# lucasjinreal/yolov7_d2

Hardware: NVIDIA H100
Metric: images/sec (640x640) YOLOX-s fwd+bwd (higher is better)
Workload: dtype bf16

## Files before the change

yolov7_d2_b200/csrc/conv_api.cu:

```cuda
#include "conv_gemm.cuh"
#include "host_common.cuh"
#include "wgrad_gemm.cuh"

#include <algorithm>
#include <cstring>

namespace yb {

template <int BN, int BK>
static int launch_conv_inst(const CUtensorMap& tmA, const CUtensorMap& tmB, const ConvGemmParams& p, dim3 grid, cudaStream_t st) {
  using Cfg = ConvGemmCfg<BN, BK>;
  const bool ext = p.epi_mode >= EPI_BF16_AFFINE;
  const int phases = p.num_phases == 4 ? 4 : 1;
  const int m_tiles = grid.x * phases, n_tiles = grid.y;
  const int occ = conv_min_ctas(BN, BK);
  const bool xpose = p.epi_mode == EPI_F32_BIAS && p.out_sc == 1;
  const int fixed = ConvEpiCfg<BN>::kStageBytes + (xpose ? kXposeBytes : 0);
  const int budget = (occ == 1 ? 212 : 104) * 1024 - 1024 - fixed;
  int slots_kb = budget / Cfg::kStageBytes;
  const int num_kb = phases == 4 ? p.cin_blocks : p.num_taps * p.cin_blocks;
  int kbs = 1;
  if (BK <= 32)
    for (int t = 1; t <= num_kb; ++t)
      if (num_kb % t == 0 && t * BK <= 144 && 2 * t <= slots_kb) kbs = t;
  int pst = slots_kb / kbs;
  if (pst > kMaxStagesP) pst = kMaxStagesP;
  if (pst < 2) pst = 2;
  const int smem = pst * kbs * Cfg::kStageBytes + 1024 + fixed;
  static PerDevice<int> smem_limit(0);
  YB_CHECK_CUDA(raise_smem_limit(smem_limit, smem, conv_gemm_persistent_kernel<BN, BK, false>, conv_gemm_persistent_kernel<BN, BK, true>));
  int groups = (occ * sm_count()) / n_tiles;
  if (groups < 1) groups = 1;
  if (groups > m_tiles) groups = m_tiles;
  if (phases == 4 && groups > 1 && groups % 2 == 0) --groups;
  ConvGemmParams pp = p;
  pp.xpose = xpose ? 1 : 0;
  if (ext)
    launch_k(conv_gemm_persistent_kernel<BN, BK, true>, groups * n_tiles, kConvThreadsP, smem, st, tmA, tmB, pp, pst, kbs, n_tiles, m_tiles);
  else
    launch_k(conv_gemm_persistent_kernel<BN, BK, false>, groups * n_tiles, kConvThreadsP, smem, st, tmA, tmB, pp, pst, kbs, n_tiles, m_tiles);
  YB_CHECK_CUDA(cudaGetLastError());
  return 0;
}

static int launch_conv(int bn, int bk, const CUtensorMap& tmA, const CUtensorMap& tmB, const ConvGemmParams& p, dim3 grid, cudaStream_t st) {
#define YB_CASE(BN, BK) \
  if (bn == BN && bk == BK) return launch_conv_inst<BN, BK>(tmA, tmB, p, grid, st);
  YB_CASE(16, 16) YB_CASE(16, 32) YB_CASE(16, 64)
  YB_CASE(32, 16) YB_CASE(32, 32) YB_CASE(32, 64)
  YB_CASE(64, 16) YB_CASE(64, 32) YB_CASE(64, 64)
  YB_CASE(128, 16) YB_CASE(128, 32) YB_CASE(128, 64)
#undef YB_CASE
  return fail(YB200_ERR_UNSUPPORTED, "no conv_gemm instantiation for BLOCK_N=%d BLOCK_K=%d", bn, bk);
}

static int pick_block_k(int c) { return c % 64 == 0 ? 64 : (c % 32 == 0 ? 32 : (c % 16 == 0 ? 16 : 0)); }
static int pick_block_n(int c) { return c > 64 ? 128 : (c > 32 ? 64 : (c > 16 ? 32 : 16)); }

static int check_arg(const yb200_act* a, const char* who, const char* arg) {
  char name[96];
  snprintf(name, sizeof(name), "%s %s", who, arg);
  return check_act(a, name);
}
// ... 676 lines not shown
```

yolov7_d2_b200/csrc/conv_gemm.cuh:

```cuda
#pragma once
#include <cuda_fp16.h>

#include "sm90.cuh"

namespace yb {

constexpr int kMaxTaps = 54;

enum EpiMode : int {
  EPI_BF16 = 0,
  EPI_F16 = 1,
  EPI_F16_STATS = 2,
  EPI_F32_BIAS = 3,
  EPI_BF16_BN_SILU = 4,
  EPI_BF16_AFFINE = 5,
  EPI_BF16_BIAS_GELU = 6,
  EPI_BF16_GELU_BWD = 7,
  EPI_BF16_BIAS_RELU = 8,
  EPI_BF16_RELU_BWD = 9,
};

__device__ __forceinline__ bool epi_has_stats(int mode, const double* stat_sum) {
  return mode == EPI_F16_STATS || ((mode == EPI_BF16_GELU_BWD || mode == EPI_BF16_RELU_BWD) && stat_sum != nullptr);
}
// ... 59 lines not shown
    ntaps = p.phase_tap[ph + 1] - tap0;
    oph = ph >> 1;
    opw = ph & 1;
  } else {
    m = wi; tap0 = 0; ntaps = p.num_taps; oph = opw = 0;
  }
}

template <int BLOCK_N, int BLOCK_K>
struct ConvGemmCfg {
  static constexpr int kSwizzle = BLOCK_K * 2;
  static constexpr int kABytes = 128 * BLOCK_K * 2;
  static constexpr int kBBytes = BLOCK_N * BLOCK_K * 2;
  static constexpr int kStageBytes = kABytes + kBBytes;
  static_assert(BLOCK_K == 16 || BLOCK_K == 32 || BLOCK_K == 64, "BLOCK_K");
  static_assert(BLOCK_N == 16 || BLOCK_N == 32 || BLOCK_N == 64 || BLOCK_N == 128, "BLOCK_N");
  static_assert(kABytes % (8 * kSwizzle) == 0 && kStageBytes % (8 * kSwizzle) == 0, "tiles must start on a swizzle-pattern boundary");
};

__device__ __forceinline__ uint32_t pack_f16x2(float lo, float hi) {
  __half2 v = __floats2half2_rn(lo, hi);
  return *reinterpret_cast<uint32_t*>(&v);
}
__device__ __forceinline__ void store_f16x8(__half* dst, const float* v) {
  uint4 u;
  u.x = pack_f16x2(v[0], v[1]);
  u.y = pack_f16x2(v[2], v[3]);
  u.z = pack_f16x2(v[4], v[5]);
  u.w = pack_f16x2(v[6], v[7]);
  *reinterpret_cast<uint4*>(dst) = u;
}
__device__ __forceinline__ void store_bf16x8(__nv_bfloat16* dst, const float* v) {
  uint4 u;
  u.x = pack_bf16x2(v[0], v[1]);
  u.y = pack_bf16x2(v[2], v[3]);
  u.z = pack_bf16x2(v[4], v[5]);
  u.w = pack_bf16x2(v[6], v[7]);
  *reinterpret_cast<uint4*>(dst) = u;
}

template <int BLOCK_N>
__device__ __forceinline__ void stage_col_params(const ConvGemmParams& p, int col0, float (*s_col)[BLOCK_N]) {
  const float* sh = p.shift ? p.shift : p.bias;
  for (int i = threadIdx.x; i < BLOCK_N; i += blockDim.x) {
    const bool ok = col0 + i < p.cout;
    s_col[0][i] = (ok && p.scale) ? p.scale[col0 + i] : 1.f;
    s_col[1][i] = (ok && sh) ? sh[col0 + i] : 0.f;
  }
}

constexpr int kXposeWarpFloats = 32 * 33 + 64;
constexpr int kXposeBytes = 8 * kXposeWarpFloats * 4;

template <int CH, bool EXT = true>
__device__ __forceinline__ void conv_epilogue_chunk(const ConvGemmParams& p, float (&v)[CH], bool valid, long long pix_off, long long add_off,
                                                    int cbase, int lane, float* part_sum, float* part_sq, bool accumulate,
                                                    const float* col_scale, const float* col_shift, float* xp = nullptr) {
  if (p.epi_mode == EPI_F32_BIAS) {
    if (xp != nullptr) {
      long long* s_off = reinterpret_cast<long long*>(xp + 32 * 33);
#pragma unroll
      for (int i = 0; i < CH; ++i) xp[lane * 33 + i] = v[i] + col_shift[i];
      s_off[lane] = valid ? pix_off : -1;
      __syncwarp();
      float* o = reinterpret_cast<float*>(p.out) + cbase + lane;
      const bool colok = lane < CH && cbase + lane < p.cout;
#pragma unroll 8
      for (int r = 0; r < 32; ++r) {
        const long long off = s_off[r];
        if (off >= 0 && colok) o[off] = xp[r * 33 + lane];
      }
      __syncwarp();
      return;
    }
    if (valid) {
      float* o = reinterpret_cast<float*>(p.out) + pix_off;
#pragma unroll
      for (int i = 0; i < CH; ++i)
        if (cbase + i < p.cout) o[(long long)(cbase + i) * p.out_sc] = v[i] + col_shift[i];
    }
    return;
  }
  if (p.epi_mode == EPI_BF16_BN_SILU) {
#pragma unroll
    for (int i = 0; i < CH; i += 4) {
      const float4 sc = *reinterpret_cast<const float4*>(col_scale + i), sh = *reinterpret_cast<const float4*>(col_shift + i);
      const float u0 = fmaf(v[i], sc.x, sh.x), u1 = fmaf(v[i + 1], sc.y, sh.y), u2 = fmaf(v[i + 2], sc.z, sh.z), u3 = fmaf(v[i + 3], sc.w, sh.w);
      v[i] = bf16_round(__fdividef(u0, 1.f + __expf(-u0)));
      v[i + 1] = bf16_round(__fdividef(u1, 1.f + __expf(-u1)));
      v[i + 2] = bf16_round(__fdividef(u2, 1.f + __expf(-u2)));
      v[i + 3] = bf16_round(__fdividef(u3, 1.f + __expf(-u3)));
    }
  }
  if constexpr (EXT) {
    if (p.epi_mode == EPI_BF16_AFFINE) {
      if (p.scale != nullptr) {
  #pragma unroll
        for (int i = 0; i < CH; i += 4) {
          const float4 sc = *reinterpret_cast<const float4*>(col_scale + i);
          v[i] *= sc.x; v[i + 1] *= sc.y; v[i + 2] *= sc.z; v[i + 3] *= sc.w;
        }
      }
      if (p.shift != nullptr) {
  #pragma unroll
        for (int i = 0; i < CH; i += 4) {
          const float4 sh = *reinterpret_cast<const float4*>(col_shift + i);
          v[i] += sh.x; v[i + 1] += sh.y; v[i + 2] += sh.z; v[i + 3] += sh.w;
        }
      }
    }
    if (p.epi_mode == EPI_BF16_BIAS_RELU) {
  #pragma unroll
      for (int i = 0; i < CH; i += 4) {
        const float4 sh = *reinterpret_cast<const float4*>(col_shift + i);
        v[i] = fmaxf(v[i] + sh.x, 0.f); v[i + 1] = fmaxf(v[i + 1] + sh.y, 0.f);
        v[i + 2] = fmaxf(v[i + 2] + sh.z, 0.f); v[i + 3] = fmaxf(v[i + 3] + sh.w, 0.f);
// ... 21 lines not shown
      }
      if (p.aux_out != nullptr && valid) {
        __nv_bfloat16* o = p.aux_out + pix_off + cbase;
  #pragma unroll
        for (int i = 0; i < CH; i += 8)
          if (cbase + i < p.cout) store_bf16x8(o + i, v + i);
      }
  #pragma unroll
      for (int i = 0; i < CH; ++i) v[i] = gelu_erf(v[i]);
    }
    if (p.epi_mode == EPI_BF16_GELU_BWD && valid) {
      const __nv_bfloat16* a = p.aux_in + pix_off + cbase;
  #pragma unroll
      for (int i = 0; i < CH; i += 8) {
        if (cbase + i < p.cout) {
          const uint4 u = *reinterpret_cast<const uint4*>(a + i);
          v[i + 0] *= gelu_erf_grad(bf16_lo(u.x)); v[i + 1] *= gelu_erf_grad(bf16_hi(u.x));
          v[i + 2] *= gelu_erf_grad(bf16_lo(u.y)); v[i + 3] *= gelu_erf_grad(bf16_hi(u.y));
          v[i + 4] *= gelu_erf_grad(bf16_lo(u.z)); v[i + 5] *= gelu_erf_grad(bf16_hi(u.z));
          v[i + 6] *= gelu_erf_grad(bf16_lo(u.w)); v[i + 7] *= gelu_erf_grad(bf16_hi(u.w));
        }
      }
    }
  }
  if (p.addend != nullptr && valid) {
    const __nv_bfloat16* a = p.addend + add_off + cbase;
#pragma unroll
    for (int i = 0; i < CH; i += 8) {
      if (cbase + i < p.cout) {
        const uint4 u = *reinterpret_cast<const uint4*>(a + i);
        v[i + 0] += bf16_lo(u.x); v[i + 1] += bf16_hi(u.x);
        v[i + 2] += bf16_lo(u.y); v[i + 3] += bf16_hi(u.y);
        v[i + 4] += bf16_lo(u.z); v[i + 5] += bf16_hi(u.z);
        v[i + 6] += bf16_lo(u.w); v[i + 7] += bf16_hi(u.w);
      }
    }
  }
  const bool f16 = p.epi_mode == EPI_F16 || p.epi_mode == EPI_F16_STATS;
  const bool need_vals = p.epi_mode == EPI_F16_STATS || (EXT && p.stat_sum != nullptr);
  if (f16) {
    uint32_t pk[CH / 2];
#pragma unroll
    for (int i = 0; i < CH; i += 2) pk[i >> 1] = pack_f16x2(v[i], v[i + 1]);
    if (valid) {
      __half* o = reinterpret_cast<__half*>(p.out) + pix_off + cbase;
#pragma unroll
      for (int i = 0; i < CH; i += 8)
        if (cbase + i < p.cout) *reinterpret_cast<uint4*>(o + i) = make_uint4(pk[i >> 1], pk[(i >> 1) + 1], pk[(i >> 1) + 2], pk[(i >> 1) + 3]);
    }
    if (need_vals) {
#pragma unroll
      for (int i = 0; i < CH; i += 2) {
        __half2 h;
        *reinterpret_cast<uint32_t*>(&h) = pk[i >> 1];
        const float2 f = __half22float2(h);
        v[i] = valid ? f.x : 0.f;
        v[i + 1] = valid ? f.y : 0.f;
      }
    }
  } else {
    uint32_t pk[CH / 2];
#pragma unroll
    for (int i = 0; i < CH; i += 2) pk[i >> 1] = pack_bf16x2(v[i], v[i + 1]);
    if (valid) {
      __nv_bfloat16* o = reinterpret_cast<__nv_bfloat16*>(p.out) + pix_off + cbase;
#pragma unroll
      for (int i = 0; i < CH; i += 8)
        if (cbase + i < p.cout) *reinterpret_cast<uint4*>(o + i) = make_uint4(pk[i >> 1], pk[(i >> 1) + 1], pk[(i >> 1) + 2], pk[(i >> 1) + 3]);
    }
    if (need_vals) {
#pragma unroll
      for (int i = 0; i < CH; i += 2) {
        v[i] = valid ? bf16_lo(pk[i >> 1]) : 0.f;
        v[i + 1] = valid ? bf16_hi(pk[i >> 1]) : 0.f;
      }
    }
  }
  if (p.epi_mode == EPI_F16_STATS) {
    float sq[CH];
#pragma unroll
    for (int i = 0; i < CH; ++i) sq[i] = v[i] * v[i];
    float cs, cq;
    if constexpr (CH == 32) { cs = warp_colsum32(v, lane); cq = warp_colsum32(sq, lane); }
    else { cs = warp_colsum16(v, lane); cq = warp_colsum16(sq, lane); }
    if (lane < CH) {
      part_sum[lane] = accumulate ? part_sum[lane] + cs : cs;
      part_sq[lane] = accumulate ? part_sq[lane] + cq : cq;
    }
  } else if (EXT && (p.epi_mode == EPI_BF16_GELU_BWD || p.epi_mode == EPI_BF16_RELU_BWD) && p.stat_sum != nullptr) {
    float cs;
    if constexpr (CH == 32) cs = warp_colsum32(v, lane);
    else cs = warp_colsum16(v, lane);
    if (lane < CH) part_sum[lane] = accumulate ? part_sum[lane] + cs : cs;
  }
}

constexpr int kMaxStagesP = 8;
constexpr int kConvThreadsP = 288;

template <int BLOCK_N>
struct ConvEpiCfg {
  static constexpr int kCols = BLOCK_N <= 64 ? (BLOCK_N < 32 ? BLOCK_N : 32) : 64;
  static_assert(BLOCK_N % kCols == 0, "staging rounds must cover the column tile");
  static constexpr int kPitch = kCols + 4;
  static constexpr int kHalves = BLOCK_N >= 32 ? 2 : 1;
  static constexpr int kChunk = kCols / kHalves;
  static constexpr int kStageBytes = 2 * 64 * kPitch * 4;
};

__host__ __device__ constexpr int conv_min_ctas(int block_n, int block_k) { return (block_n >= 128 || block_k == 16) ? 1 : 2; }

template <int BLOCK_N, int BLOCK_K, bool EXT>
__global__ void __launch_bounds__(kConvThreadsP, conv_min_ctas(BLOCK_N, BLOCK_K))
conv_gemm_persistent_kernel(const __grid_constant__ CUtensorMap tmA, const __grid_constant__ CUtensorMap tmB,
                            const __grid_constant__ ConvGemmParams p, int num_stages, int kb_per_slot, int n_tiles, int m_tiles) {
  using Cfg = ConvGemmCfg<BLOCK_N, BLOCK_K>;
  using Epi = ConvEpiCfg<BLOCK_N>;
  constexpr int CH = Epi::kChunk;
  extern __shared__ uint8_t smem_dyn[];
  __shared__ __align__(8) uint64_t s_bar[2 * kMaxStagesP];
  __shared__ float s_part[4][2][BLOCK_N];
  __shared__ __align__(16) float s_col[2][BLOCK_N];

  const int warp = warp_id_uniform();
  const int lane = threadIdx.x & 31;
  const uint32_t smem_base = (smem_u32(smem_dyn) + 1023u) & ~1023u;
  uint8_t* const smem_al = smem_dyn + (smem_base - smem_u32(smem_dyn));
  const int ring_bytes = num_stages * kb_per_slot * Cfg::kStageBytes;
  const uint32_t bar_full = smem_u32(&s_bar[0]);
  const uint32_t bar_empty = smem_u32(&s_bar[kMaxStagesP]);

  const int n_tile = blockIdx.x % n_tiles;
  const int group = blockIdx.x / n_tiles;
  const int groups = gridDim.x / n_tiles;
  const int col0 = n_tile * BLOCK_N;
  const int log_tw = p.log_tw, log_th = p.log_th;

  if (threadIdx.x == 0) {
    for (int s = 0; s < num_stages; ++s) {
      mbar_init(bar_full + 8 * s, 1);
      mbar_init(bar_empty + 8 * s, 2);
    }
    mbar_fence_init();
  }
  for (int i = threadIdx.x; i < 4 * 2 * BLOCK_N; i += blockDim.x) (&s_part[0][0][0])[i] = 0.f;
  pdl_sync();
  stage_col_params<BLOCK_N>(p, col0, s_col);
  __syncthreads();

  if (warp == 8) {
    if (elect_one()) {
      tma_prefetch_desc(&tmA);
      tma_prefetch_desc(&tmB);
      int stage = 0;
      uint32_t phase = 0;
      for (int wi = group; wi < m_tiles; wi += groups) {
        int m, tap, ntaps, oph, opw;
        conv_decode_work(p, wi, m, tap, ntaps, oph, opw);
        const int num_kb = ntaps * p.cin_blocks;
        int t = m;
        const int tw = t % p.tiles_w;
        t /= p.tiles_w;
        const int th = t % p.tiles_h;
        const int tn = t / p.tiles_h;
        const int w0 = tw << log_tw, h0 = th << log_th, n0 = tn << (7 - log_tw - log_th);
// ... 5 lines not shown
          for (int j = 0; j < kb_per_slot; ++j) {
            const uint32_t sa = smem_base + (stage * kb_per_slot + j) * Cfg::kStageBytes;
            const ConvTap& tp = p.taps[tap];
            tma_load_5d(sa, &tmA, full, tp.c0 + cb * BLOCK_K, w0 + tp.dw, tp.p, h0 + tp.dh, n0);
            tma_load_2d(sa + Cfg::kABytes, &tmB, full, tp.kb + cb * BLOCK_K, col0 + n0 * p.b_img_rows);
            if (++cb == p.cin_blocks) { cb = 0; ++tap; }
          }
          if (++stage == num_stages) { stage = 0; phase ^= 1u; }
        }
      }
    }
  } else if (warp < 8) {
    const int g = warp >> 2;
    const int wl = warp & 3;
    const int q = 2 * g + (wl & 1);
    const int half = wl >> 1;
    const int mrow = q * 32 + lane;
    const int xl = mrow & ((1 << log_tw) - 1);
    const int yl = (mrow >> log_tw) & ((1 << log_th) - 1);
    const int nl = mrow >> (log_tw + log_th);
    float* const stg = reinterpret_cast<float*>(smem_al + ring_bytes) + g * 64 * Epi::kPitch;
    float* xp = nullptr;
    if (p.xpose) xp = reinterpret_cast<float*>(smem_al + ring_bytes + Epi::kStageBytes) + warp * kXposeWarpFloats;
    constexpr uint32_t lcode = gmma_layout_code(Cfg::kSwizzle);
    constexpr uint32_t sbo = 8 * Cfg::kSwizzle;
    float acc[BLOCK_N / 2];
#pragma unroll
    for (int i = 0; i < BLOCK_N / 2; ++i) acc[i] = 0.f;
    wgmma_fence_operand(acc);
    int stage = 0;
    uint32_t phase = 0;
    for (int wi = group; wi < m_tiles; wi += groups) {
      int m, tap, ntaps, oph, opw;
      conv_decode_work(p, wi, m, tap, ntaps, oph, opw);
      const int num_kb = ntaps * p.cin_blocks;
      int j = 0, prev = -1;
      for (int kb = 0; kb < num_kb; ++kb) {
        if (j == 0) mbar_wait(bar_full + 8 * stage, phase);
        const uint32_t sa = smem_base + (stage * kb_per_slot + j) * Cfg::kStageBytes + g * 64 * Cfg::kSwizzle;
        const uint32_t sb = smem_base + (stage * kb_per_slot + j) * Cfg::kStageBytes + Cfg::kABytes;
        wgmma_fence_operand(acc);
        wgmma_fence();
#pragma unroll
        for (int k = 0; k < BLOCK_K / 16; ++k)
          Wgmma<BLOCK_N>::template mma<0, 0>(acc, gmma_desc(sa + k * 32, 16, sbo, lcode), gmma_desc(sb + k * 32, 16, sbo, lcode), (kb | k) != 0 ? 1u : 0u);
        wgmma_commit();
        wgmma_wait<1>();
        wgmma_fence_operand(acc);
        mbar_arrive_if(bar_empty + 8 * prev, j == 0 && prev >= 0 && (threadIdx.x & 127) == 0);
        if (++j == kb_per_slot) {
          j = 0;
          prev = stage;
          if (++stage == num_stages) { stage = 0; phase ^= 1u; }
        }
      }
      wgmma_wait<0>();
      wgmma_fence_operand(acc);
      mbar_arrive_if(bar_empty + 8 * prev, (threadIdx.x & 127) == 0);

      int t = m;
      const int tw = t % p.tiles_w;
      t /= p.tiles_w;
      const int th = t % p.tiles_h;
      const int tn = t / p.tiles_h;
      const int x = (tw << log_tw) + xl, y = (th << log_th) + yl, n = (tn << (7 - log_tw - log_th)) + nl;
      const bool valid = (x < p.w_valid) && (y < p.h_valid) && (n < p.n_valid);
      const long long pix_off = (long long)n * p.out_sn + (long long)(y * p.out_mh + oph) * p.out_sh +
                                (long long)(x * p.out_mw + opw) * p.out_sw;
      const long long add_off = (long long)n * p.add_sn + (long long)(y * p.out_mh + oph) * p.add_sh +
                                (long long)(x * p.out_mw + opw) * p.add_sw;
      float* const r0 = stg + (16 * wl + (lane >> 2)) * Epi::kPitch + 2 * (lane & 3);
      float* const r1 = r0 + 8 * Epi::kPitch;
      const float* const row_src = stg + ((wl & 1) * 32 + lane) * Epi::kPitch + half * CH;
#pragma unroll 1
      for (int r = 0; r < BLOCK_N / Epi::kCols; ++r) {
        named_bar_sync(1 + g, 128);
#pragma unroll
        for (int i = 0; i < BLOCK_N / 8; ++i) {
          if (i / (Epi::kCols / 8) == r) {
            const int c = (i % (Epi::kCols / 8)) * 8;
            *reinterpret_cast<float2*>(r0 + c) = make_float2(acc[4 * i], acc[4 * i + 1]);
            *reinterpret_cast<float2*>(r1 + c) = make_float2(acc[4 * i + 2], acc[4 * i + 3]);
          }
        }
        named_bar_sync(1 + g, 128);
        const int c = r * Epi::kCols + half * CH;
        if (half < Epi::kHalves && col0 + c < p.cout) {
          float v[CH];
#pragma unroll
          for (int i = 0; i < CH; i += 4) {
            const float4 f = *reinterpret_cast<const float4*>(row_src + i);
            v[i] = f.x; v[i + 1] = f.y; v[i + 2] = f.z; v[i + 3] = f.w;
          }
          conv_epilogue_chunk<CH, EXT>(p, v, valid, pix_off, add_off, col0 + c, lane, &s_part[q][0][c], &s_part[q][1][c], true, &s_col[0][c],
                                       &s_col[1][c], xp);
        }
      }
    }
  }

  __syncthreads();
  if (EXT ? epi_has_stats(p.epi_mode, p.stat_sum) : p.epi_mode == EPI_F16_STATS) {
    for (int e = threadIdx.x; e < BLOCK_N && col0 + e < p.cout; e += blockDim.x) {
      const float s1 = (s_part[0][0][e] + s_part[1][0][e]) + (s_part[2][0][e] + s_part[3][0][e]);
      const float s2 = (s_part[0][1][e] + s_part[1][1][e]) + (s_part[2][1][e] + s_part[3][1][e]);
      const int ch = p.stat_fold > 0 ? (col0 + e) % p.stat_fold : col0 + e;
      atomicAdd(p.stat_sum + ch, static_cast<double>(s1));
      if (p.stat_sq != nullptr) atomicAdd(p.stat_sq + ch, static_cast<double>(s2));
    }
  }
}

}
```

yolov7_d2_b200/csrc/host_common.cu:

```cuda
#include "host_common.cuh"

#include <mutex>

namespace yb {

static thread_local char g_err[1024] = "";

char* err_buf() { return g_err; }

int fail(int code, const char* fmt, ...) {
  va_list ap;
  va_start(ap, fmt);
  vsnprintf(g_err, sizeof(g_err), fmt, ap);
  va_end(ap);
  return code;
}

int current_device() {
  int dev = 0;
  if (cudaGetDevice(&dev) != cudaSuccess) return 0;
  return dev;
}

int sm_count() {
// ... 61 lines not shown
  YB_REQUIRE(r == CUDA_SUCCESS, YB200_ERR_CUDA,
             "cuTensorMapEncodeTiled(act n=%d h=%d w=%d pitch=%d box=%d,%d,%d,%d) failed: %d", a.n, a.h, a.w, a.c_pitch,
             box_c, tw, th, tn, static_cast<int>(r));
  return 0;
}

int make_mat_map(CUtensorMap* m, const void* ptr, long long rows, long long cols, int box_rows, int box_cols) {
  EncodeTiledFn fn = encode_fn();
  YB_REQUIRE(fn != nullptr, YB200_ERR_CUDA, "cuTensorMapEncodeTiled entry point not available");
  YB_REQUIRE((reinterpret_cast<uintptr_t>(ptr) & 15) == 0 && cols % 8 == 0, YB200_ERR_INVALID,
             "matrix must be 16B aligned with a row length multiple of 8");
  cuuint64_t gdim[2] = {static_cast<cuuint64_t>(cols), static_cast<cuuint64_t>(rows)};
  cuuint64_t gstr[1] = {static_cast<cuuint64_t>(cols) * 2};
  cuuint32_t box[2] = {static_cast<cuuint32_t>(box_cols), static_cast<cuuint32_t>(box_rows)};
  cuuint32_t estr[2] = {1, 1};
  CUresult r = fn(m, CU_TENSOR_MAP_DATA_TYPE_BFLOAT16, 2, const_cast<void*>(ptr), gdim, gstr, box, estr,
                  CU_TENSOR_MAP_INTERLEAVE_NONE, swizzle_for(box_cols * 2), CU_TENSOR_MAP_L2_PROMOTION_L2_128B,
                  CU_TENSOR_MAP_FLOAT_OOB_FILL_NONE);
  YB_REQUIRE(r == CUDA_SUCCESS, YB200_ERR_CUDA, "cuTensorMapEncodeTiled(mat %lldx%lld box %dx%d) failed: %d", rows, cols,
             box_rows, box_cols, static_cast<int>(r));
  return 0;
}

void choose_tile(int n, int h, int w, int npix, int* log_tw, int* log_th) {
  const int lp = ilog2(npix);
  long long best = -1;
  int bw = 0, bh = 0;
  for (int lw = lp; lw >= 0; --lw) {
    for (int lh = lp - lw; lh >= 0; --lh) {
      const int tw = 1 << lw, th = 1 << lh, tn = npix >> (lw + lh);
      const long long cost = 1LL * ceil_div(w, tw) * tw * ceil_div(h, th) * th * ceil_div(n, tn) * tn;
      if (best < 0 || cost < best) {
        best = cost; bw = lw; bh = lh;
      }
    }
  }
  *log_tw = bw;
  *log_th = bh;
}

}

extern "C" int yb200_version(void) { return YB200_VERSION; }
extern "C" const char* yb200_last_error(void) { return yb::err_buf(); }
```

yolov7_d2_b200/csrc/host_common.cuh:

```cuda
#pragma once
#include <cuda.h>
#include <cuda_runtime.h>
#include <stdarg.h>
#include <stdio.h>
#include <string.h>

#include <utility>

#include "../../include/yb200.h"

namespace yb {

char* err_buf();
int fail(int code, const char* fmt, ...);
int sm_count();
int current_device();
template <typename T>
struct PerDevice {
  T v[64];
  T init;
  bool used[64];
  explicit PerDevice(T init_value) : init(init_value) { memset(used, 0, sizeof(used)); }
  T& cur() {
    const int d = current_device() & 63;
// ... 10 lines not shown
  ((e = e == cudaSuccess ? cudaFuncSetAttribute(kernels, cudaFuncAttributeMaxDynamicSharedMemorySize, bytes) : e), ...);
  if (e == cudaSuccess) cur = bytes;
  return e;
}

#define YB_CHECK_CUDA(expr)                                                                      \
  do {                                                                                           \
    cudaError_t _e = (expr);                                                                     \
    if (_e != cudaSuccess) return yb::fail(YB200_ERR_CUDA, "%s: %s", #expr, cudaGetErrorString(_e)); \
  } while (0)
#define YB_REQUIRE(cond, code, ...) \
  do {                              \
    if (!(cond)) return yb::fail(code, __VA_ARGS__); \
  } while (0)

inline cudaStream_t as_stream(void* s) { return reinterpret_cast<cudaStream_t>(s); }

int check_act(const yb200_act* a, const char* name, int mult = 8);
inline bool same_shape(const yb200_act* a, const yb200_act* b) { return a->n == b->n && a->h == b->h && a->w == b->w && a->c == b->c; }
inline bool same_geometry(const yb200_act* a, const yb200_act* b) { return same_shape(a, b) && a->c_pitch == b->c_pitch; }

int make_act_map(CUtensorMap* m, const yb200_act& a, bool space_to_depth, int box_c, int tw, int th, int tn);
int make_mat_map(CUtensorMap* m, const void* ptr, long long rows, long long cols, int box_rows, int box_cols);

void choose_tile(int n, int h, int w, int npix, int* log_tw, int* log_th);

template <typename... K, typename... A>
inline cudaError_t launch_k_opt(bool pdl, void (*kernel)(K...), dim3 grid, dim3 block, size_t smem, cudaStream_t st, A&&... args) {
  cudaLaunchConfig_t cfg = {};
  cfg.gridDim = grid;
  cfg.blockDim = block;
  cfg.dynamicSmemBytes = smem;
  cfg.stream = st;
  cudaLaunchAttribute at[1];
  at[0].id = cudaLaunchAttributeProgrammaticStreamSerialization;
  at[0].val.programmaticStreamSerializationAllowed = 1;
  cfg.attrs = at;
  cfg.numAttrs = pdl ? 1 : 0;
  return cudaLaunchKernelEx(&cfg, kernel, std::forward<A>(args)...);
}
template <typename... K, typename... A>
inline cudaError_t launch_k(void (*kernel)(K...), dim3 grid, dim3 block, size_t smem, cudaStream_t st, A&&... args) {
  return launch_k_opt(true, kernel, grid, block, smem, st, std::forward<A>(args)...);
}

inline int ceil_div(int a, int b) { return (a + b - 1) / b; }
// ... 4 lines not shown
```

yolov7_d2_b200/csrc/sm90.cuh:

```cuda
#pragma once
#include <cuda.h>
#include <cuda_runtime.h>
#include <cuda_bf16.h>
#include <stdint.h>
#include <stdio.h>

namespace yb {

__device__ __forceinline__ void pdl_sync() {
  asm volatile("griddepcontrol.wait;" ::: "memory");
  asm volatile("griddepcontrol.launch_dependents;" ::: "memory");
}

__device__ __forceinline__ uint32_t smem_u32(const void* p) {
  return static_cast<uint32_t>(__cvta_generic_to_shared(p));
}

__device__ __forceinline__ bool elect_one() {
  uint32_t pred = 0;
  asm volatile(
      "{\n\t.reg .pred P;\n\t"
      "elect.sync _|P, 0xffffffff;\n\t"
      "selp.u32 %0, 1, 0, P;\n\t}\n"
      : "=r"(pred));
// ... 37 lines not shown
__device__ __forceinline__ int warp_id_uniform() { return __shfl_sync(0xffffffffu, static_cast<int>(threadIdx.x >> 5), 0); }

__device__ __forceinline__ void tma_prefetch_desc(const CUtensorMap* m) {
  asm volatile("prefetch.tensormap [%0];" ::"l"(reinterpret_cast<uint64_t>(m)) : "memory");
}
__device__ __forceinline__ void tma_load_2d(uint32_t dst, const CUtensorMap* m, uint32_t bar, int c0,
                                            int c1) {
  asm volatile(
      "cp.async.bulk.tensor.2d.shared::cluster.global.mbarrier::complete_tx::bytes [%0], [%1, {%3, "
      "%4}], [%2];"
      ::"r"(dst), "l"(reinterpret_cast<uint64_t>(m)), "r"(bar), "r"(c0), "r"(c1)
      : "memory");
}
__device__ __forceinline__ void tma_load_5d(uint32_t dst, const CUtensorMap* m, uint32_t bar, int c0,
                                            int c1, int c2, int c3, int c4) {
  asm volatile(
      "cp.async.bulk.tensor.5d.shared::cluster.global.mbarrier::complete_tx::bytes [%0], [%1, {%3, "
      "%4, %5, %6, %7}], [%2];"
      ::"r"(dst), "l"(reinterpret_cast<uint64_t>(m)), "r"(bar), "r"(c0), "r"(c1), "r"(c2), "r"(c3),
      "r"(c4)
      : "memory");
}

__device__ __forceinline__ void fence_proxy_async_smem() { asm volatile("fence.proxy.async.shared::cta;" ::: "memory"); }

__host__ __device__ constexpr uint32_t gmma_layout_code(int swizzle_bytes) {
  return swizzle_bytes == 128 ? 1u : swizzle_bytes == 64 ? 2u : swizzle_bytes == 32 ? 3u : 0u;
}
__device__ __forceinline__ uint64_t gmma_desc(uint32_t saddr, uint32_t lbo_bytes, uint32_t sbo_bytes, uint32_t layout_code) {
  uint64_t d = 0;
  d |= static_cast<uint64_t>((saddr & 0x3FFFFu) >> 4);
  d |= static_cast<uint64_t>((lbo_bytes >> 4) & 0x3FFFu) << 16;
  d |= static_cast<uint64_t>((sbo_bytes >> 4) & 0x3FFFu) << 32;
  d |= static_cast<uint64_t>(layout_code) << 62;
  return d;
}
__device__ __forceinline__ void wgmma_fence() { asm volatile("wgmma.fence.sync.aligned;" ::: "memory"); }
__device__ __forceinline__ void wgmma_commit() { asm volatile("wgmma.commit_group.sync.aligned;" ::: "memory"); }
template <int N>
__device__ __forceinline__ void wgmma_wait() { asm volatile("wgmma.wait_group.sync.aligned %0;" ::"n"(N) : "memory"); }
template <int R>
__device__ __forceinline__ void wgmma_fence_operand(float (&d)[R]) {
#pragma unroll
  for (int i = 0; i < R; ++i) asm volatile("" : "+f"(d[i])::"memory");
}

template <int N>
// ... 113 lines not shown
```

Baseline: 2037.

## Route 16-bit conv epilogue through swizzled smem with TMA stores and residual loads

Result: faster. 2332, median of 6 (+14.5%).

```diff
diff --git a/yolov7_d2_b200/csrc/conv_api.cu b/yolov7_d2_b200/csrc/conv_api.cu
--- a/yolov7_d2_b200/csrc/conv_api.cu
+++ b/yolov7_d2_b200/csrc/conv_api.cu
@@ -6,11 +6,39 @@
 #include <cstring>
 
 namespace yb {
+
+static int make_out_maps(ConvOutMaps* om, const ConvGemmParams& p, int bn) {
+  YB_REQUIRE(p.out_sc == 1, YB200_ERR_INVALID, "conv: a 16-bit output needs channel stride 1");
+  int hx, hy, hn;
+  conv_half_offset(p.log_tw, p.log_th, hx, hy, hn);
+  const int tw = 1 << p.log_tw, th = 1 << p.log_th, tn = 128 >> (p.log_tw + p.log_th);
+  const int bw = hx ? tw / 2 : tw, bh = hy ? th / 2 : th, bnn = hn ? tn / 2 : tn;
+  const int box_c = bn < 64 ? bn : 64;
+  for (int ph = 0; ph < (p.num_phases == 4 ? 4 : 1); ++ph) {
+    const int oph = ph >> 1, opw = ph & 1;
+    const char* out = static_cast<const char*>(p.out) + 2 * (oph * p.out_sh + opw * p.out_sw);
+    int rc = make_pix_map(&om->out[ph], out, p.cout, p.w_valid, p.h_valid, p.n_valid, p.out_mw * p.out_sw, p.out_mh * p.out_sh, p.out_sn, box_c,
+                          bw, bh, bnn);
+    if (rc) return rc;
+    if (p.addend == nullptr) continue;
+    const char* add = reinterpret_cast<const char*>(p.addend) + 2 * (oph * p.add_sh + opw * p.add_sw);
+    rc = make_pix_map(&om->add[ph], add, p.cout, p.w_valid, p.h_valid, p.n_valid, p.out_mw * p.add_sw, p.out_mh * p.add_sh, p.add_sn, box_c, bw,
+                      bh, bnn);
+    if (rc) return rc;
+  }
+  return 0;
+}
 
 template <int BN, int BK>
 static int launch_conv_inst(const CUtensorMap& tmA, const CUtensorMap& tmB, const ConvGemmParams& p, dim3 grid, cudaStream_t st) {
   using Cfg = ConvGemmCfg<BN, BK>;
   const bool ext = p.epi_mode >= EPI_BF16_AFFINE;
+  ConvOutMaps om;
+  memset(&om, 0, sizeof(om));
+  if (!ext && p.epi_mode != EPI_F32_BIAS) {
+    const int rc = make_out_maps(&om, p, BN);
+    if (rc) return rc;
+  }
   const int phases = p.num_phases == 4 ? 4 : 1;
   const int m_tiles = grid.x * phases, n_tiles = grid.y;
   const int occ = conv_min_ctas(BN, BK);
@@ -36,9 +64,9 @@
   ConvGemmParams pp = p;
   pp.xpose = xpose ? 1 : 0;
   if (ext)
-    launch_k(conv_gemm_persistent_kernel<BN, BK, true>, groups * n_tiles, kConvThreadsP, smem, st, tmA, tmB, pp, pst, kbs, n_tiles, m_tiles);
+    launch_k(conv_gemm_persistent_kernel<BN, BK, true>, groups * n_tiles, kConvThreadsP, smem, st, tmA, tmB, pp, om, pst, kbs, n_tiles, m_tiles);
   else
-    launch_k(conv_gemm_persistent_kernel<BN, BK, false>, groups * n_tiles, kConvThreadsP, smem, st, tmA, tmB, pp, pst, kbs, n_tiles, m_tiles);
+    launch_k(conv_gemm_persistent_kernel<BN, BK, false>, groups * n_tiles, kConvThreadsP, smem, st, tmA, tmB, pp, om, pst, kbs, n_tiles, m_tiles);
   YB_CHECK_CUDA(cudaGetLastError());
   return 0;
 }
diff --git a/yolov7_d2_b200/csrc/conv_gemm.cuh b/yolov7_d2_b200/csrc/conv_gemm.cuh
--- a/yolov7_d2_b200/csrc/conv_gemm.cuh
+++ b/yolov7_d2_b200/csrc/conv_gemm.cuh
@@ -105,14 +105,6 @@
   __half2 v = __floats2half2_rn(lo, hi);
   return *reinterpret_cast<uint32_t*>(&v);
 }
-__device__ __forceinline__ void store_f16x8(__half* dst, const float* v) {
-  uint4 u;
-  u.x = pack_f16x2(v[0], v[1]);
-  u.y = pack_f16x2(v[2], v[3]);
-  u.z = pack_f16x2(v[4], v[5]);
-  u.w = pack_f16x2(v[6], v[7]);
-  *reinterpret_cast<uint4*>(dst) = u;
-}
 __device__ __forceinline__ void store_bf16x8(__nv_bfloat16* dst, const float* v) {
   uint4 u;
   u.x = pack_bf16x2(v[0], v[1]);
@@ -137,8 +129,8 @@
 
 template <int CH, bool EXT = true>
 __device__ __forceinline__ void conv_epilogue_chunk(const ConvGemmParams& p, float (&v)[CH], bool valid, long long pix_off, long long add_off,
-                                                    int cbase, int lane, float* part_sum, float* part_sq, bool accumulate,
-                                                    const float* col_scale, const float* col_shift, float* xp = nullptr) {
+                                                    int cbase, int lane, float* part_sum, bool accumulate, const float* col_scale,
+                                                    const float* col_shift, float* xp = nullptr) {
   if (p.epi_mode == EPI_F32_BIAS) {
     if (xp != nullptr) {
       long long* s_off = reinterpret_cast<long long*>(xp + 32 * 33);
@@ -164,17 +156,6 @@
     }
     return;
   }
-  if (p.epi_mode == EPI_BF16_BN_SILU) {
-#pragma unroll
-    for (int i = 0; i < CH; i += 4) {
-      const float4 sc = *reinterpret_cast<const float4*>(col_scale + i), sh = *reinterpret_cast<const float4*>(col_shift + i);
-      const float u0 = fmaf(v[i], sc.x, sh.x), u1 = fmaf(v[i + 1], sc.y, sh.y), u2 = fmaf(v[i + 2], sc.z, sh.z), u3 = fmaf(v[i + 3], sc.w, sh.w);
-      v[i] = bf16_round(__fdividef(u0, 1.f + __expf(-u0)));
-      v[i + 1] = bf16_round(__fdividef(u1, 1.f + __expf(-u1)));
-      v[i + 2] = bf16_round(__fdividef(u2, 1.f + __expf(-u2)));
-      v[i + 3] = bf16_round(__fdividef(u3, 1.f + __expf(-u3)));
-    }
-  }
   if constexpr (EXT) {
     if (p.epi_mode == EPI_BF16_AFFINE) {
       if (p.scale != nullptr) {
@@ -242,43 +223,19 @@
         }
       }
     }
-  }
-  if (p.addend != nullptr && valid) {
-    const __nv_bfloat16* a = p.addend + add_off + cbase;
-#pragma unroll
-    for (int i = 0; i < CH; i += 8) {
-      if (cbase + i < p.cout) {
-        const uint4 u = *reinterpret_cast<const uint4*>(a + i);
-        v[i + 0] += bf16_lo(u.x); v[i + 1] += bf16_hi(u.x);
-        v[i + 2] += bf16_lo(u.y); v[i + 3] += bf16_hi(u.y);
-        v[i + 4] += bf16_lo(u.z); v[i + 5] += bf16_hi(u.z);
-        v[i + 6] += bf16_lo(u.w); v[i + 7] += bf16_hi(u.w);
-      }
-    }
-  }
-  const bool f16 = p.epi_mode == EPI_F16 || p.epi_mode == EPI_F16_STATS;
-  const bool need_vals = p.epi_mode == EPI_F16_STATS || (EXT && p.stat_sum != nullptr);
-  if (f16) {
-    uint32_t pk[CH / 2];
-#pragma unroll
-    for (int i = 0; i < CH; i += 2) pk[i >> 1] = pack_f16x2(v[i], v[i + 1]);
-    if (valid) {
-      __half* o = reinterpret_cast<__half*>(p.out) + pix_off + cbase;
-#pragma unroll
-      for (int i = 0; i < CH; i += 8)
-        if (cbase + i < p.cout) *reinterpret_cast<uint4*>(o + i) = make_uint4(pk[i >> 1], pk[(i >> 1) + 1], pk[(i >> 1) + 2], pk[(i >> 1) + 3]);
-    }
-    if (need_vals) {
-#pragma unroll
-      for (int i = 0; i < CH; i += 2) {
-        __half2 h;
-        *reinterpret_cast<uint32_t*>(&h) = pk[i >> 1];
-        const float2 f = __half22float2(h);
-        v[i] = valid ? f.x : 0.f;
-        v[i + 1] = valid ? f.y : 0.f;
-      }
-    }
-  } else {
+      if (p.addend != nullptr && valid) {
+      const __nv_bfloat16* a = p.addend + add_off + cbase;
+#pragma unroll
+      for (int i = 0; i < CH; i += 8) {
+        if (cbase + i < p.cout) {
+          const uint4 u = *reinterpret_cast<const uint4*>(a + i);
+          v[i + 0] += bf16_lo(u.x); v[i + 1] += bf16_hi(u.x);
+          v[i + 2] += bf16_lo(u.y); v[i + 3] += bf16_hi(u.y);
+          v[i + 4] += bf16_lo(u.z); v[i + 5] += bf16_hi(u.z);
+          v[i + 6] += bf16_lo(u.w); v[i + 7] += bf16_hi(u.w);
+        }
+      }
+    }
     uint32_t pk[CH / 2];
 #pragma unroll
     for (int i = 0; i < CH; i += 2) pk[i >> 1] = pack_bf16x2(v[i], v[i + 1]);
@@ -288,30 +245,17 @@
       for (int i = 0; i < CH; i += 8)
         if (cbase + i < p.cout) *reinterpret_cast<uint4*>(o + i) = make_uint4(pk[i >> 1], pk[(i >> 1) + 1], pk[(i >> 1) + 2], pk[(i >> 1) + 3]);
     }
-    if (need_vals) {
+    if ((p.epi_mode == EPI_BF16_GELU_BWD || p.epi_mode == EPI_BF16_RELU_BWD) && p.stat_sum != nullptr) {
 #pragma unroll
       for (int i = 0; i < CH; i += 2) {
         v[i] = valid ? bf16_lo(pk[i >> 1]) : 0.f;
         v[i + 1] = valid ? bf16_hi(pk[i >> 1]) : 0.f;
       }
-    }
-  }
-  if (p.epi_mode == EPI_F16_STATS) {
-    float sq[CH];
-#pragma unroll
-    for (int i = 0; i < CH; ++i) sq[i] = v[i] * v[i];
-    float cs, cq;
-    if constexpr (CH == 32) { cs = warp_colsum32(v, lane); cq = warp_colsum32(sq, lane); }
-    else { cs = warp_colsum16(v, lane); cq = warp_colsum16(sq, lane); }
-    if (lane < CH) {
-      part_sum[lane] = accumulate ? part_sum[lane] + cs : cs;
-      part_sq[lane] = accumulate ? part_sq[lane] + cq : cq;
-    }
-  } else if (EXT && (p.epi_mode == EPI_BF16_GELU_BWD || p.epi_mode == EPI_BF16_RELU_BWD) && p.stat_sum != nullptr) {
-    float cs;
-    if constexpr (CH == 32) cs = warp_colsum32(v, lane);
-    else cs = warp_colsum16(v, lane);
-    if (lane < CH) part_sum[lane] = accumulate ? part_sum[lane] + cs : cs;
+      float cs;
+      if constexpr (CH == 32) cs = warp_colsum32(v, lane);
+      else cs = warp_colsum16(v, lane);
+      if (lane < CH) part_sum[lane] = accumulate ? part_sum[lane] + cs : cs;
+    }
   }
 }
 
@@ -328,17 +272,44 @@
   static constexpr int kStageBytes = 2 * 64 * kPitch * 4;
 };
 
+template <int BLOCK_N>
+struct ConvTmaEpiCfg {
+  static constexpr int kBoxCols = BLOCK_N < 64 ? BLOCK_N : 64;
+  static constexpr int kBoxes = BLOCK_N / kBoxCols;
+  static constexpr int kRowBytes = 2 * kBoxCols;
+  static constexpr int kBoxBytes = 64 * kRowBytes;
+  static constexpr int kBufBytes = kBoxes * kBoxBytes;
+  static constexpr int kBufs = 2 * 2 * kBufBytes <= ConvEpiCfg<BLOCK_N>::kStageBytes ? 2 : 1;
+  static_assert(2 * kBufs * kBufBytes <= ConvEpiCfg<BLOCK_N>::kStageBytes, "output tiles must fit in the staging tile's bytes");
+};
+
+struct ConvOutMaps {
+  CUtensorMap out[4];
+  CUtensorMap add[4];
+};
+
 __host__ __device__ constexpr int conv_min_ctas(int block_n, int block_k) { return (block_n >= 128 || block_k == 16) ? 1 : 2; }
+
+__host__ __device__ inline void conv_half_offset(int log_tw, int log_th, int& dx, int& dy, int& dn) {
+  const int log_tn = 7 - log_tw - log_th;
+  dx = dy = dn = 0;
+  if (log_tn > 0) dn = 1 << (log_tn - 1);
+  else if (log_th > 0) dy = 1 << (log_th - 1);
+  else dx = 1 << (log_tw - 1);
+}
 
 template <int BLOCK_N, int BLOCK_K, bool EXT>
 __global__ void __launch_bounds__(kConvThreadsP, conv_min_ctas(BLOCK_N, BLOCK_K))
 conv_gemm_persistent_kernel(const __grid_constant__ CUtensorMap tmA, const __grid_constant__ CUtensorMap tmB,
-                            const __grid_constant__ ConvGemmParams p, int num_stages, int kb_per_slot, int n_tiles, int m_tiles) {
+                            const __grid_constant__ ConvGemmParams p, const __grid_constant__ ConvOutMaps om, int num_stages, int kb_per_slot,
+                            int n_tiles, int m_tiles) {
   using Cfg = ConvGemmCfg<BLOCK_N, BLOCK_K>;
   using Epi = ConvEpiCfg<BLOCK_N>;
+  using TE = ConvTmaEpiCfg<BLOCK_N>;
+  static_assert(Cfg::kStageBytes % (8 * TE::kRowBytes) == 0, "output tiles must start on a swizzle-pattern boundary");
   constexpr int CH = Epi::kChunk;
   extern __shared__ uint8_t smem_dyn[];
-  __shared__ __align__(8) uint64_t s_bar[2 * kMaxStagesP];
+  __shared__ __align__(8) uint64_t s_bar[2 * kMaxStagesP + 4];
   __shared__ float s_part[4][2][BLOCK_N];
   __shared__ __align__(16) float s_col[2][BLOCK_N];
 
@@ -349,6 +320,8 @@
   const int ring_bytes = num_stages * kb_per_slot * Cfg::kStageBytes;
   const uint32_t bar_full = smem_u32(&s_bar[0]);
   const uint32_t bar_empty = smem_u32(&s_bar[kMaxStagesP]);
+  const uint32_t bar_add = smem_u32(&s_bar[2 * kMaxStagesP]);
+  const bool tma_epi = !EXT && p.epi_mode != EPI_F32_BIAS;
 
   const int n_tile = blockIdx.x % n_tiles;
   const int group = blockIdx.x / n_tiles;
@@ -361,6 +334,7 @@
       mbar_init(bar_full + 8 * s, 1);
       mbar_init(bar_empty + 8 * s, 2);
     }
+    for (int s = 0; s < 4; ++s) mbar_init(bar_add + 8 * s, 1);
     mbar_fence_init();
   }
   for (int i = threadIdx.x; i < 4 * 2 * BLOCK_N; i += blockDim.x) (&s_part[0][0][0])[i] = 0.f;
@@ -412,6 +386,19 @@
     float* const stg = reinterpret_cast<float*>(smem_al + ring_bytes) + g * 64 * Epi::kPitch;
     float* xp = nullptr;
     if (p.xpose) xp = reinterpret_cast<float*>(smem_al + ring_bytes + Epi::kStageBytes) + warp * kXposeWarpFloats;
+    const bool leader = (threadIdx.x & 127) == 0;
+    const bool add_tile = tma_epi && p.addend != nullptr;
+    const uint32_t obuf = smem_base + ring_bytes + g * TE::kBufs * TE::kBufBytes;
+    const int srow = 16 * wl + (lane & 7) + 8 * ((lane >> 3) & 1);
+    const uint32_t srow_off = srow * TE::kRowBytes;
+    const uint32_t schunk = (lane >> 4) ^ ((srow_off >> 7) & (TE::kRowBytes / 16 - 1));
+    int hx, hy, hn;
+    conv_half_offset(log_tw, log_th, hx, hy, hn);
+    hx *= g; hy *= g; hn *= g;
+    if (tma_epi && leader) {
+      tma_prefetch_desc(&om.out[0]);
+      if (add_tile) tma_prefetch_desc(&om.add[0]);
+    }
     constexpr uint32_t lcode = gmma_layout_code(Cfg::kSwizzle);
     constexpr uint32_t sbo = 8 * Cfg::kSwizzle;
     float acc[BLOCK_N / 2];
@@ -420,10 +407,27 @@
     wgmma_fence_operand(acc);
     int stage = 0;
     uint32_t phase = 0;
-    for (int wi = group; wi < m_tiles; wi += groups) {
+    int it = 0;
+    for (int wi = group; wi < m_tiles; wi += groups, ++it) {
       int m, tap, ntaps, oph, opw;
       conv_decode_work(p, wi, m, tap, ntaps, oph, opw);
       const int num_kb = ntaps * p.cin_blocks;
+      int t = m;
+      const int tw = t % p.tiles_w;
+      t /= p.tiles_w;
+      const int th = t % p.tiles_h;
+      const int tn = t / p.tiles_h;
+      const int w0 = tw << log_tw, h0 = th << log_th, n0 = tn << (7 - log_tw - log_th);
+      const int pm = p.num_phases == 4 ? 2 * oph + opw : 0;
+      const int slot = TE::kBufs == 2 ? (it & 1) : 0;
+      const uint32_t buf = obuf + slot * TE::kBufBytes;
+      const uint32_t abar = bar_add + 8 * (2 * g + slot);
+      if (add_tile && leader) {
+        if (TE::kBufs == 1) bulk_wait_read<0>();
+        mbar_expect_tx(abar, TE::kBufBytes);
+#pragma unroll
+        for (int b = 0; b < TE::kBoxes; ++b) tma_load_4d(buf + b * TE::kBoxBytes, &om.add[pm], abar, col0 + 64 * b, w0 + hx, h0 + hy, n0 + hn);
+      }
       int j = 0, prev = -1;
       for (int kb = 0; kb < num_kb; ++kb) {
         if (j == 0) mbar_wait(bar_full + 8 * stage, phase);
@@ -448,45 +452,130 @@
       wgmma_fence_operand(acc);
       mbar_arrive_if(bar_empty + 8 * prev, (threadIdx.x & 127) == 0);
 
-      int t = m;
-      const int tw = t % p.tiles_w;
-      t /= p.tiles_w;
-      const int th = t % p.tiles_h;
-      const int tn = t / p.tiles_h;
-      const int x = (tw << log_tw) + xl, y = (th << log_th) + yl, n = (tn << (7 - log_tw - log_th)) + nl;
-      const bool valid = (x < p.w_valid) && (y < p.h_valid) && (n < p.n_valid);
-      const long long pix_off = (long long)n * p.out_sn + (long long)(y * p.out_mh + oph) * p.out_sh +
-                                (long long)(x * p.out_mw + opw) * p.out_sw;
-      const long long add_off = (long long)n * p.add_sn + (long long)(y * p.out_mh + oph) * p.add_sh +
-                                (long long)(x * p.out_mw + opw) * p.add_sw;
-      float* const r0 = stg + (16 * wl + (lane >> 2)) * Epi::kPitch + 2 * (lane & 3);
-      float* const r1 = r0 + 8 * Epi::kPitch;
-      const float* const row_src = stg + ((wl & 1) * 32 + lane) * Epi::kPitch + half * CH;
+      if (tma_epi) {
+        if (TE::kBufs == 1 && !add_tile) {
+          if (leader) bulk_wait_read<0>();
+          named_bar_sync(1 + g, 128);
+        }
+        if (p.epi_mode == EPI_BF16_BN_SILU) {
+#pragma unroll
+          for (int i = 0; i < BLOCK_N / 8; ++i) {
+            const float2 sc = *reinterpret_cast<const float2*>(&s_col[0][8 * i + 2 * (lane & 3)]);
+            const float2 sh = *reinterpret_cast<const float2*>(&s_col[1][8 * i + 2 * (lane & 3)]);
+#pragma unroll
+            for (int e = 0; e < 4; ++e) {
+              const float u = fmaf(acc[4 * i + e], (e & 1) ? sc.y : sc.x, (e & 1) ? sh.y : sh.x);
+              acc[4 * i + e] = bf16_round(__fdividef(u, 1.f + __expf(-u)));
+            }
+          }
+        }
+        if (add_tile) {
+          mbar_wait(abar, (it / TE::kBufs) & 1);
+#pragma unroll
+          for (int i = 0; i < BLOCK_N / 8; i += 2) {
+            uint32_t a[4];
+            ldmatrix_x4(buf + (i >> 3) * TE::kBoxBytes + srow_off + (((i & 7) ^ schunk) << 4), a[0], a[1], a[2], a[3]);
+#pragma unroll
+            for (int r = 0; r < 4; ++r) {
+              acc[4 * i + 2 * r] += bf16_lo(a[r]);
+              acc[4 * i + 2 * r + 1] += bf16_hi(a[r]);
+            }
+          }
+        }
+        uint32_t pk[BLOCK_N / 4];
+        if (p.epi_mode == EPI_F16 || p.epi_mode == EPI_F16_STATS) {
+#pragma unroll
+          for (int i = 0; i < BLOCK_N / 4; ++i) pk[i] = pack_f16x2(acc[2 * i], acc[2 * i + 1]);
+        } else {
+#pragma unroll
+          for (int i = 0; i < BLOCK_N / 4; ++i) pk[i] = pack_bf16x2(acc[2 * i], acc[2 * i + 1]);
+        }
+#pragma unroll
+        for (int i = 0; i < BLOCK_N / 8; i += 2)
+          stmatrix_x4(buf + (i >> 3) * TE::kBoxBytes + srow_off + (((i & 7) ^ schunk) << 4), pk[2 * i], pk[2 * i + 1], pk[2 * i + 2], pk[2 * i + 3]);
+        fence_proxy_async_smem();
+        if (TE::kBufs == 2 && leader) bulk_wait_read<0>();
+        named_bar_sync(1 + g, 128);
+        if (leader) {
+#pragma unroll
+          for (int b = 0; b < TE::kBoxes; ++b) tma_store_4d(&om.out[pm], buf + b * TE::kBoxBytes, col0 + 64 * b, w0 + hx, h0 + hy, n0 + hn);
+          bulk_commit();
+        }
+        if (p.epi_mode == EPI_F16_STATS) {
+          const bool valid = w0 + xl < p.w_valid && h0 + yl < p.h_valid && n0 + nl < p.n_valid;
+          const uint32_t row = (wl & 1) * 32 + lane;
+          const uint32_t rxor = ((row * TE::kRowBytes) >> 7) & (TE::kRowBytes / 16 - 1);
 #pragma unroll 1
-      for (int r = 0; r < BLOCK_N / Epi::kCols; ++r) {
-        named_bar_sync(1 + g, 128);
-#pragma unroll
-        for (int i = 0; i < BLOCK_N / 8; ++i) {
-          if (i / (Epi::kCols / 8) == r) {
-            const int c = (i % (Epi::kCols / 8)) * 8;
-            *reinterpret_cast<float2*>(r0 + c) = make_float2(acc[4 * i], acc[4 * i + 1]);
-            *reinterpret_cast<float2*>(r1 + c) = make_float2(acc[4 * i + 2], acc[4 * i + 3]);
+          for (int r = 0; r < BLOCK_N / Epi::kCols; ++r) {
+            const int c = r * Epi::kCols + half * CH;
+            if (half < Epi::kHalves && col0 + c < p.cout) {
+              float v[CH], sq[CH];
+#pragma unroll
+              for (int i = 0; i < CH; i += 8) {
+                const int cc = c + i;
+                uint4 u;
+                asm volatile("ld.shared.v4.u32 {%0, %1, %2, %3}, [%4];"
+                             : "=r"(u.x), "=r"(u.y), "=r"(u.z), "=r"(u.w)
+                             : "r"(buf + (cc / TE::kBoxCols) * TE::kBoxBytes + row * TE::kRowBytes + ((((cc % TE::kBoxCols) >> 3) ^ rxor) << 4))
+                             : "memory");
+                const uint32_t w4[4] = {u.x, u.y, u.z, u.w};
+#pragma unroll
+                for (int j = 0; j < 4; ++j) {
+                  __half2 hv;
+                  *reinterpret_cast<uint32_t*>(&hv) = w4[j];
+                  const float2 fv = __half22float2(hv);
+                  v[i + 2 * j] = valid ? fv.x : 0.f;
+                  v[i + 2 * j + 1] = valid ? fv.y : 0.f;
+                }
+              }
+#pragma unroll
+              for (int i = 0; i < CH; ++i) sq[i] = v[i] * v[i];
+              float cs, cq;
+              if constexpr (CH == 32) { cs = warp_colsum32(v, lane); cq = warp_colsum32(sq, lane); }
+              else { cs = warp_colsum16(v, lane); cq = warp_colsum16(sq, lane); }
+              if (lane < CH) {
+                s_part[q][0][c + lane] += cs;
+                s_part[q][1][c + lane] += cq;
+              }
+            }
           }
         }
-        named_bar_sync(1 + g, 128);
-        const int c = r * Epi::kCols + half * CH;
-        if (half < Epi::kHalves && col0 + c < p.cout) {
-          float v[CH];
-#pragma unroll
-          for (int i = 0; i < CH; i += 4) {
-            const float4 f = *reinterpret_cast<const float4*>(row_src + i);
-            v[i] = f.x; v[i + 1] = f.y; v[i + 2] = f.z; v[i + 3] = f.w;
+      } else {
+        const int x = w0 + xl, y = h0 + yl, n = n0 + nl;
+        const bool valid = (x < p.w_valid) && (y < p.h_valid) && (n < p.n_valid);
+        const long long pix_off = (long long)n * p.out_sn + (long long)(y * p.out_mh + oph) * p.out_sh +
+                                  (long long)(x * p.out_mw + opw) * p.out_sw;
+        const long long add_off = (long long)n * p.add_sn + (long long)(y * p.out_mh + oph) * p.add_sh +
+                                  (long long)(x * p.out_mw + opw) * p.add_sw;
+        float* const r0 = stg + (16 * wl + (lane >> 2)) * Epi::kPitch + 2 * (lane & 3);
+        float* const r1 = r0 + 8 * Epi::kPitch;
+        const float* const row_src = stg + ((wl & 1) * 32 + lane) * Epi::kPitch + half * CH;
+#pragma unroll 1
+        for (int r = 0; r < BLOCK_N / Epi::kCols; ++r) {
+          named_bar_sync(1 + g, 128);
+#pragma unroll
+          for (int i = 0; i < BLOCK_N / 8; ++i) {
+            if (i / (Epi::kCols / 8) == r) {
+              const int c = (i % (Epi::kCols / 8)) * 8;
+              *reinterpret_cast<float2*>(r0 + c) = make_float2(acc[4 * i], acc[4 * i + 1]);
+              *reinterpret_cast<float2*>(r1 + c) = make_float2(acc[4 * i + 2], acc[4 * i + 3]);
+            }
           }
-          conv_epilogue_chunk<CH, EXT>(p, v, valid, pix_off, add_off, col0 + c, lane, &s_part[q][0][c], &s_part[q][1][c], true, &s_col[0][c],
-                                       &s_col[1][c], xp);
-        }
-      }
-    }
+          named_bar_sync(1 + g, 128);
+          const int c = r * Epi::kCols + half * CH;
+          if (half < Epi::kHalves && col0 + c < p.cout) {
+            float v[CH];
+#pragma unroll
+            for (int i = 0; i < CH; i += 4) {
+              const float4 f = *reinterpret_cast<const float4*>(row_src + i);
+              v[i] = f.x; v[i + 1] = f.y; v[i + 2] = f.z; v[i + 3] = f.w;
+            }
+            conv_epilogue_chunk<CH, EXT>(p, v, valid, pix_off, add_off, col0 + c, lane, &s_part[q][0][c], true, &s_col[0][c], &s_col[1][c], xp);
+          }
+        }
+      }
+    }
+    if (tma_epi && leader) bulk_wait_all();
   }
 
   __syncthreads();
diff --git a/yolov7_d2_b200/csrc/host_common.cu b/yolov7_d2_b200/csrc/host_common.cu
--- a/yolov7_d2_b200/csrc/host_common.cu
+++ b/yolov7_d2_b200/csrc/host_common.cu
@@ -107,6 +107,23 @@
   return 0;
 }
 
+int make_pix_map(CUtensorMap* m, const void* base, int c, int w, int h, int n, long long sx, long long sy, long long sn, int box_c, int bw, int bh,
+                 int bn) {
+  EncodeTiledFn fn = encode_fn();
+  YB_REQUIRE(fn != nullptr, YB200_ERR_CUDA, "cuTensorMapEncodeTiled entry point not available");
+  YB_REQUIRE((reinterpret_cast<uintptr_t>(base) & 15) == 0 && sx % 8 == 0 && sy % 8 == 0 && sn % 8 == 0, YB200_ERR_INVALID,
+             "16-bit pixel view must start 16B aligned with strides that are multiples of 8 elements (strides %lld, %lld, %lld)", sx, sy, sn);
+  cuuint64_t gdim[4] = {static_cast<cuuint64_t>(c), static_cast<cuuint64_t>(w), static_cast<cuuint64_t>(h), static_cast<cuuint64_t>(n)};
+  cuuint64_t gstr[3] = {static_cast<cuuint64_t>(sx) * 2, static_cast<cuuint64_t>(sy) * 2, static_cast<cuuint64_t>(sn) * 2};
+  cuuint32_t box[4] = {static_cast<cuuint32_t>(box_c), static_cast<cuuint32_t>(bw), static_cast<cuuint32_t>(bh), static_cast<cuuint32_t>(bn)};
+  cuuint32_t estr[4] = {1, 1, 1, 1};
+  CUresult r = fn(m, CU_TENSOR_MAP_DATA_TYPE_UINT16, 4, const_cast<void*>(base), gdim, gstr, box, estr, CU_TENSOR_MAP_INTERLEAVE_NONE,
+                  swizzle_for(box_c * 2), CU_TENSOR_MAP_L2_PROMOTION_L2_128B, CU_TENSOR_MAP_FLOAT_OOB_FILL_NONE);
+  YB_REQUIRE(r == CUDA_SUCCESS, YB200_ERR_CUDA, "cuTensorMapEncodeTiled(pixels c=%d w=%d h=%d n=%d box=%d,%d,%d,%d) failed: %d", c, w, h, n,
+             box_c, bw, bh, bn, static_cast<int>(r));
+  return 0;
+}
+
 void choose_tile(int n, int h, int w, int npix, int* log_tw, int* log_th) {
   const int lp = ilog2(npix);
   long long best = -1;
diff --git a/yolov7_d2_b200/csrc/host_common.cuh b/yolov7_d2_b200/csrc/host_common.cuh
--- a/yolov7_d2_b200/csrc/host_common.cuh
+++ b/yolov7_d2_b200/csrc/host_common.cuh
@@ -56,6 +56,8 @@
 
 int make_act_map(CUtensorMap* m, const yb200_act& a, bool space_to_depth, int box_c, int tw, int th, int tn);
 int make_mat_map(CUtensorMap* m, const void* ptr, long long rows, long long cols, int box_rows, int box_cols);
+int make_pix_map(CUtensorMap* m, const void* base, int c, int w, int h, int n, long long sx, long long sy, long long sn, int box_c, int bw, int bh,
+                 int bn);
 
 void choose_tile(int n, int h, int w, int npix, int* log_tw, int* log_th);
 
diff --git a/yolov7_d2_b200/csrc/sm90.cuh b/yolov7_d2_b200/csrc/sm90.cuh
--- a/yolov7_d2_b200/csrc/sm90.cuh
+++ b/yolov7_d2_b200/csrc/sm90.cuh
@@ -83,7 +83,34 @@
       : "memory");
 }
 
+__device__ __forceinline__ void tma_load_4d(uint32_t dst, const CUtensorMap* m, uint32_t bar, int c0, int c1, int c2, int c3) {
+  asm volatile(
+      "cp.async.bulk.tensor.4d.shared::cluster.global.mbarrier::complete_tx::bytes [%0], [%1, {%3, %4, %5, %6}], [%2];"
+      ::"r"(dst), "l"(reinterpret_cast<uint64_t>(m)), "r"(bar), "r"(c0), "r"(c1), "r"(c2), "r"(c3)
+      : "memory");
+}
+__device__ __forceinline__ void tma_store_4d(const CUtensorMap* m, uint32_t src, int c0, int c1, int c2, int c3) {
+  asm volatile("cp.async.bulk.tensor.4d.global.shared::cta.bulk_group [%0, {%2, %3, %4, %5}], [%1];"
+               ::"l"(reinterpret_cast<uint64_t>(m)), "r"(src), "r"(c0), "r"(c1), "r"(c2), "r"(c3)
+               : "memory");
+}
+__device__ __forceinline__ void bulk_commit() { asm volatile("cp.async.bulk.commit_group;" ::: "memory"); }
+template <int N>
+__device__ __forceinline__ void bulk_wait_read() { asm volatile("cp.async.bulk.wait_group.read %0;" ::"n"(N) : "memory"); }
+__device__ __forceinline__ void bulk_wait_all() { asm volatile("cp.async.bulk.wait_group 0;" ::: "memory"); }
+
 __device__ __forceinline__ void fence_proxy_async_smem() { asm volatile("fence.proxy.async.shared::cta;" ::: "memory"); }
+
+__device__ __forceinline__ void stmatrix_x4(uint32_t addr, uint32_t r0, uint32_t r1, uint32_t r2, uint32_t r3) {
+  asm volatile("stmatrix.sync.aligned.m8n8.x4.shared.b16 [%0], {%1, %2, %3, %4};" ::"r"(addr), "r"(r0), "r"(r1), "r"(r2), "r"(r3)
+               : "memory");
+}
+__device__ __forceinline__ void ldmatrix_x4(uint32_t addr, uint32_t& r0, uint32_t& r1, uint32_t& r2, uint32_t& r3) {
+  asm volatile("ldmatrix.sync.aligned.m8n8.x4.shared.b16 {%0, %1, %2, %3}, [%4];"
+               : "=r"(r0), "=r"(r1), "=r"(r2), "=r"(r3)
+               : "r"(addr)
+               : "memory");
+}
 
 __host__ __device__ constexpr uint32_t gmma_layout_code(int swizzle_bytes) {
   return swizzle_bytes == 128 ? 1u : swizzle_bytes == 64 ? 2u : swizzle_bytes == 32 ? 3u : 0u;
```
